# flanglet/kanzi-go

Measured on AMD Instinct MI355X. Metric: encode+decode MB/s (round trip of the whole stream, uncompressed 10^6 B per second), higher is better.
Workload: dtype u8

## Files before the change

### kanzi-go_amd/csrc/ans1.hip

```cpp
#include "bits.h"

#define KNZ_ANS1_CHUNK (4u << 20)
#define KNZ_ANS1_LR 11
#define KNZ_ANS1_SCALE 2048
#define KNZ_ANS1_LDS_MAX_CHUNKS 1280u
#define KNZ_ANS1_CTXHDR_BYTES 448
#define KNZ_ANS1_U0_CAP (256 * KNZ_ANS1_CTXHDR_BYTES + 64)
#define KNZ_ANS1_U1_OFF KNZ_ANS1_U0_CAP
#define KNZ_ANS1_PAY_OFF (KNZ_ANS1_U0_CAP + 64)
#define KNZ_ANS1_PAY_CAP (((KNZ_ANS1_CHUNK / 8) * 11) + 64)
#define KNZ_ANS1_SLOT (KNZ_ANS1_PAY_OFF + KNZ_ANS1_PAY_CAP + 64)
#define KNZ_ANS1_CUM_STRIDE 257
#define KNZ_ANS1_PAYRING 8192
#define KNZ_ANS1_RING 2048

struct Ans1Args {
    const uint64_t* blk_off;
    const uint32_t* blk_len;
    uint32_t chunks_per_block;
    uint32_t nslots;
    uint8_t* scratch;
    uint32_t* unit_bits;
    uint32_t* unit_src;
    uint32_t* freqs;
// ... 397 lines not shown
        flushed += c0 + c1 + c2;
        wave_sync_lds();
    };
#pragma unroll
    for (int j = 0; j < KNZ_ANS1_GROUP; j++) { buf0[j].x = 0; buf0[j].y = 0xFFFFFFFFu; buf0[j].z = 0; buf0[j].w = 0; buf1[j] = buf0[j]; }
    for (uint32_t t0 = 0; t0 < steps + 2 * KNZ_ANS1_GROUP && steps; t0 += 3 * KNZ_ANS1_GROUP) {
        load_group(t0, buf2, xm2); knz_a1e_run_group<0>(st, buf0, mine);
        const uint32_t f0 = xm0;
        load_group(t0 + KNZ_ANS1_GROUP, buf0, xm0); knz_a1e_run_group<1>(st, buf1, mine);
        const uint32_t f1 = xm1;
        load_group(t0 + 2 * KNZ_ANS1_GROUP, buf1, xm1); knz_a1e_run_group<2>(st, buf2, mine);
        flush(f0, f1, xm2);
    }
    const uint32_t s1 = wave_shfl(st, 1), s2 = wave_shfl(st, 2), s3 = wave_shfl(st, 3);
    if (bad && lane == 0) a.blk_status[b] = KNZ_ERR_PROCESS_BLOCK;
    if (live && lane == 0) {
        const uint32_t end4 = n & ~3u;
        const uint32_t tail = n & 3;
        for (uint32_t i = 0; i < tail; i++) payEnd[i] = src[end4 + i];
        const uint32_t nbytes = 2 * flushed + tail;
        uint32_t w[8];
        for (int i = 0; i < 8; i++) w[i] = 0;
        KnzBitWriter bw;
        bw.init(w);
        knz_put_varint(bw, nbytes);
        bw.put(st, 32); bw.put(s1, 32); bw.put(s2, 32); bw.put(s3, 32);
        uint32_t* u1 = (uint32_t*)(slot + KNZ_ANS1_U1_OFF);
        for (int i = 0; i < 8; i++) u1[i] = knz_bswap32(w[i]);
        uint32_t* ubits = a.unit_bits + (size_t)slotId * KNZ_UNITS_PER_CHUNK;
        uint32_t* usrc = a.unit_src + (size_t)slotId * KNZ_UNITS_PER_CHUNK;
        ubits[1] = bw.pos;
        ubits[2] = 8 * nbytes;
        usrc[2] = (uint32_t)(KNZ_ANS1_PAY_OFF + KNZ_ANS1_PAY_CAP - 2 * flushed);
    }
}
#endif

struct Ans1DecArgs {
    const uint8_t* stream; uint64_t nbytes;
    const uint32_t* blk_pre_len;
    const uint8_t* blk_mode;
    const uint64_t* chunk_bit;
    const uint64_t* blk_out_off;
    uint32_t chunks_per_block;
    uint32_t nslots;
    uint32_t* dtab;
    uint32_t* info;
    uint64_t* paybit;
    int32_t* blk_status;
    uint32_t plain_loop;
    uint64_t* progress;
};

template <typename R>
__device__ static bool knz_ans1_parse_ctx(R& r, uint16_t* f, uint32_t llr, uint32_t scale, int& countOut) {
    uint8_t alpha[256];
    int count = 0;
    if (r.read(1) == 0) {
        if (r.read(1) == 1) count = 0;
        else { count = 256; if (f) for (int i = 0; i < 256; i++) alpha[i] = (uint8_t)i; }
    } else {
        const uint32_t lastMask = r.read(5);
        if (f) {
            for (uint32_t mm = 0; mm <= lastMask; mm++) {
                const uint32_t mask = r.read(8);
                for (int j = 0; j < 8; j++) if ((mask >> j) & 1) alpha[count++] = (uint8_t)(8 * mm + j);
            }
        } else {
            for (uint32_t bitsLeft = 8 * (lastMask + 1); bitsLeft > 0;) {
                const uint32_t take = bitsLeft > 32 ? 32 : bitsLeft;
                count += __popc(r.read(take));
                bitsLeft -= take;
            }
        }
    }
    countOut = count;
    if (count == 0) return true;
    const int chk = count < 64 ? 6 : 8;
    uint32_t sum = 0;
    for (int i = 1; i < count; i += chk) {
        const uint32_t logMax = r.read(llr);
        if ((1u << logMax) > scale) return false;
        const int endj = min(i + chk, count);
        if (!f) { r.skip_bits((uint32_t)(endj - i) * logMax); continue; }
        for (int j = i; j < endj; j++) {
            uint32_t fr = 1;
            if (logMax > 0) { fr = 1 + r.read(logMax); if (fr >= scale) return false; }
            f[alpha[j]] = (uint16_t)fr;
            sum += fr;
        }
    }
    if (f) {
        if (scale <= sum) return false;
        f[alpha[0]] = (uint16_t)(scale - sum);
    }
    return true;
}

template <typename R>
__device__ static bool knz_ans1_parse_header(R& r, uint16_t* freq16, uint32_t& lrOut, int& totalAlpha, uint64_t* ctxpos, bool store) {
    const uint32_t lr = 8 + r.read(3);
    lrOut = lr;
    if (lr > 16) return false;
    uint32_t llr = 3;
    while ((1u << llr) <= lr) llr++;
    const uint32_t scale = 1u << lr;
    totalAlpha = 0;
    for (int k = 0; k < 256; k++) {
        if (ctxpos && store) ctxpos[k] = r.tell();
        int count = 0;
        if (!knz_ans1_parse_ctx(r, freq16 ? freq16 + (size_t)k * 256 : nullptr, llr, scale, count)) return false;
        totalAlpha += count;
    }
    if (ctxpos && store) ctxpos[256] = r.tell();
    return true;
}

__global__ __launch_bounds__(256) void knz_ans1_dec_tables_kernel(Ans1DecArgs a, uint16_t* freq16, uint16_t* cum16, const uint64_t* ctx_bit) {
    __shared__ int s_mode;
    __shared__ uint32_t s_lr;
    __shared__ int s_total, s_badctx;
    const int tid = threadIdx.x;
    const uint32_t slotId = blockIdx.x;
    const uint32_t b = slotId / a.chunks_per_block, k = slotId % a.chunks_per_block;
    uint32_t* info = a.info + (size_t)slotId * 8;
    const uint32_t preLen = a.blk_pre_len[b];
    if (tid == 0) info[0] = 0;
    if (a.blk_status[b] != 0 || (uint64_t)k * KNZ_ANS1_CHUNK >= preLen) return;
    if ((a.blk_mode[b] & 0x80) || preLen <= 32) { if (tid == 0) info[0] = 1; return; }
    uint16_t* f16 = freq16 + (size_t)slotId * 65536;
    for (int i = tid; i < 65536; i += 256) f16[i] = 0;
    __syncthreads();
    const uint64_t* cpos = ctx_bit ? ctx_bit + (size_t)slotId * 257 : nullptr;
    if (cpos) {
        if (tid == 0) { s_total = 0; s_badctx = 0; }
        __syncthreads();
        KnzStreamReader r0;
// ... 550 lines not shown
```

### kanzi-go_amd/csrc/huffman_dec.hip

```cpp
#include "bits.h"

struct KnzStreamReader {
    const uint32_t* words;
    uint64_t nwords;
    uint64_t next;
    uint64_t win;
    uint32_t navail;
    uint32_t pre;
    __device__ __forceinline__ uint32_t ld_raw(uint64_t i) const { return i < nwords ? words[i] : 0u; }
    __device__ __forceinline__ uint32_t ld(uint64_t i) const { return knz_bswap32(ld_raw(i)); }
    __device__ __forceinline__ void init(const uint8_t* base, uint64_t nbytes, uint64_t bitpos) {
        words = (const uint32_t*)base;
        nwords = (nbytes + 3) >> 2;
        uint64_t q = bitpos >> 5;
        uint32_t off = (uint32_t)(bitpos & 31);
        win = ((uint64_t)ld(q) << 32) | ld(q + 1);
        win <<= off;
        navail = 64 - off;
        next = q + 2;
        pre = ld_raw(next);
    }
    __device__ __forceinline__ void refill() {
        if (navail <= 32) { win |= (uint64_t)knz_bswap32(pre) << (32 - navail); navail += 32; next++; pre = ld_raw(next); }
    }
    __device__ __forceinline__ uint32_t peek(uint32_t n) { refill(); return (uint32_t)(win >> (64 - n)); }
    __device__ __forceinline__ void skip(uint32_t n) { refill(); win <<= n; navail -= n; }
    __device__ __forceinline__ void consume(uint32_t n) { win <<= n; navail -= n; }
    __device__ __forceinline__ void skip_bits(uint32_t n) { if (n <= 32) skip(n); else seek(tell() + n); }
    __device__ __forceinline__ uint32_t read(uint32_t n) { uint32_t v = peek(n); win <<= n; navail -= n; return v; }
    __device__ __forceinline__ uint64_t tell() const { return (next << 5) - navail; }
    __device__ __forceinline__ void seek(uint64_t bitpos) { init((const uint8_t*)words, nwords << 2, bitpos); }
};

struct KnzWaveReader {
    const uint32_t* words;
    uint64_t nwords;
    uint64_t base;
    uint32_t w0, w1;
    uint64_t next;
    uint64_t win;
    uint32_t navail;
    __device__ __forceinline__ void stage(uint64_t b) {
        const uint64_t l = (uint64_t)lane_id();
        base = b;
        w0 = (b + l < nwords) ? words[b + l] : 0u;
        w1 = (b + 64 + l < nwords) ? words[b + 64 + l] : 0u;
    }
    __device__ __forceinline__ uint32_t ld(uint64_t i) {
        if (i < base || i >= base + 128) stage(i);
        const uint32_t k = (uint32_t)(i - base);
        const uint32_t v = k < 64 ? wave_readlane(w0, k) : wave_readlane(w1, k - 64);
        return knz_bswap32(v);
    }
    __device__ __forceinline__ void init(const uint8_t* b, uint64_t nbytes, uint64_t bitpos) {
        words = (const uint32_t*)b;
        nwords = (nbytes + 3) >> 2;
        stage(bitpos >> 5);
        seek(bitpos);
    }
    __device__ __forceinline__ void seek(uint64_t bitpos) {
        const uint64_t q = bitpos >> 5;
        const uint32_t off = (uint32_t)(bitpos & 31);
        win = ((uint64_t)ld(q) << 32) | ld(q + 1);
        win <<= off;
        navail = 64 - off;
        next = q + 2;
    }
    __device__ __forceinline__ void refill() {
        if (navail <= 32) { win |= (uint64_t)ld(next++) << (32 - navail); navail += 32; }
    }
    __device__ __forceinline__ uint32_t peek(uint32_t n) { refill(); return (uint32_t)(win >> (64 - n)); }
    __device__ __forceinline__ void skip(uint32_t n) { refill(); win <<= n; navail -= n; }
    __device__ __forceinline__ void skip_bits(uint32_t n) { if (n <= 32) skip(n); else seek(tell() + n); }
    __device__ __forceinline__ uint32_t read(uint32_t n) { uint32_t v = peek(n); win <<= n; navail -= n; return v; }
    __device__ __forceinline__ uint64_t tell() const { return (next << 5) - navail; }
};

template <typename R>
__device__ __forceinline__ uint32_t knz_read_varint(R& r) {
    uint32_t res = 0, shift = 0;
    for (int i = 0; i < 4; i++) {
        uint32_t v = r.read(8);
        res |= (v & 0x7F) << shift;
        if (v < 128) return res;
        shift += 7;
    }
    uint32_t v = r.read(8);
    return res | ((v & 0x0F) << 28);
}

template <typename R>
__device__ static bool knz_ans1_parse_header(R& r, uint16_t* freq16, uint32_t& lrOut, int& totalAlpha, uint64_t* ctxpos, bool store);

struct WalkStreamArgs {
    const uint8_t* stream; uint64_t nbytes;
    uint64_t first_bit;
    uint64_t seg_bits;
    uint32_t max_blocks;
    uint64_t* blk_bit;
    uint64_t* blk_bits;
    uint32_t* result;
};

__global__ void knz_dec_walk_stream_kernel(WalkStreamArgs a) {
    if (threadIdx.x != 0 || blockIdx.x != 0) return;
    KnzStreamReader r;
    r.init(a.stream, a.nbytes, a.first_bit);
    const uint64_t limit = a.nbytes << 3;
    uint32_t n = 0, err = 0;
    for (;;) {
        if (a.seg_bits && r.tell() >= a.first_bit + a.seg_bits) break;
        if (r.tell() + 8 > limit) { err = KNZ_ERR_PROCESS_BLOCK; break; }
        uint32_t lr = r.read(5) + 3;
        uint64_t read = 0;
        if (lr > 32) { read = (uint64_t)r.read(lr - 32) << 32; read |= r.read(32); }
        else read = r.read(lr);
        if (read == 0) break;
        if (read > ((uint64_t)1 << 34)) { err = KNZ_ERR_BLOCK_SIZE; break; }
        uint64_t pos = r.tell();
        if (pos + read > limit) { err = KNZ_ERR_PROCESS_BLOCK; break; }
        if (n >= a.max_blocks) { err = KNZ_ERR_BLOCK_SIZE; break; }
        a.blk_bit[n] = pos;
        a.blk_bits[n] = read;
        n++;
        r.seek(pos + read);
    }
    a.result[0] = n;
    a.result[1] = err;
// ... 16 lines not shown
    if (threadIdx.x != 0 || blockIdx.x != 0) return;
    KnzStreamReader r;
    r.init(a.stream, a.nbytes, a.first_bit);
    const uint64_t limit = a.nbytes << 3;
    uint64_t id = a.first_id, n = 0, end = 0;
    uint32_t seen = 0, err = 0;
    while (id < a.to) {
        const uint64_t at = r.tell();
        if (at + 8 > limit) { err = KNZ_ERR_PROCESS_BLOCK; break; }
        const uint32_t lr = r.read(5) + 3;
        uint64_t read = 0;
        if (lr > 32) { read = (uint64_t)r.read(lr - 32) << 32; read |= r.read(32); }
        else read = r.read(lr);
        const uint64_t pos = r.tell();
        if (read == 0) { end = pos; if (a.hinted && seen == 0) err = KNZ_ERR_PROCESS_BLOCK; break; }
        if (read > ((uint64_t)1 << 34)) { err = KNZ_ERR_BLOCK_SIZE; break; }
        if (pos + read > limit) { err = KNZ_ERR_PROCESS_BLOCK; break; }
        if (seen >= a.max_blocks) { err = KNZ_ERR_BLOCK_SIZE; break; }
        seen++;
        if (id >= a.from) {
            if (n < a.cap) { a.blk_bit[n * a.stride] = a.frames ? at : pos; a.blk_bits[n * a.stride] = read; }
            n++;
        }
        id++;
        r.seek(pos + read);
    }
    a.result[0] = n;
    a.result[1] = err;
    a.result[2] = end;
}

struct WalkBlocksArgs {
    const uint8_t* stream; uint64_t nbytes;
    const uint64_t* blk_bit; const uint64_t* blk_bits;
    uint32_t nblocks;
    uint32_t block_size;
    uint32_t checksum_bits;
    uint32_t entropy;
    uint32_t chunks_per_block;
    uint32_t payload_only;
    uint32_t given_len;
    uint32_t* blk_pre_len;
    uint8_t* blk_mode;
    uint8_t* blk_skip;
    uint64_t* blk_cksum;
    uint64_t* chunk_bit;
    int32_t* blk_status;
    uint64_t* blk_end_bit;
    uint32_t check_out;
    uint64_t* out_off;
    uint64_t out_base, out_stride, out_cap;
    uint32_t stream_block_size;
    uint64_t* ans1_ctx_bit;
};

template <typename R>
__device__ __forceinline__ void knz_skip_expg(R& r) {
    uint32_t w = r.peek(17);
    if (w & 0x10000) { r.skip(1); return; }
    if (w == 0) { r.skip(17); return; }
    uint32_t z = (uint32_t)__builtin_clz(w << 15);
    uint32_t lg = z & 7;
    r.skip(z + 1);
    r.skip(lg + 1);
}

#define KNZ_EXPG_WIN 12
__device__ __forceinline__ uint32_t knz_expg_lut_entry(uint32_t w) {
    uint32_t pos = 0, codes = 0;
    while (pos < KNZ_EXPG_WIN) {
        if ((w >> (KNZ_EXPG_WIN - 1 - pos)) & 1) { codes++; pos++; continue; }
        uint32_t z = 0;
        while (pos + z < KNZ_EXPG_WIN && !((w >> (KNZ_EXPG_WIN - 1 - pos - z)) & 1)) z++;
        if (pos + z >= KNZ_EXPG_WIN) break;
        const uint32_t total = z + 1 + (z & 7) + 1;
        if (pos + total > KNZ_EXPG_WIN) break;
        codes++; pos += total;
    }
    return (codes << 4) | pos;
}

struct HufDecArgs {
    const uint8_t* stream; uint64_t nbytes;
    const uint32_t* blk_pre_len;
    const uint8_t* blk_mode;
    const uint64_t* chunk_bit;
    const uint64_t* blk_out_off;
    uint32_t chunks_per_block;
    uint32_t entropy;
    uint8_t* out;
    int32_t* blk_status;
};

__global__ __launch_bounds__(64) void knz_huf_decode_kernel(HufDecArgs a, const uint8_t* only) {
    __shared__ uint16_t s_table[1 << KNZ_HUF_MAXLEN];
    __shared__ uint8_t s_len[256];
    __shared__ uint8_t s_alpha[256];
    __shared__ uint16_t s_C[256];
    __shared__ uint8_t s_symAt[256];
    __shared__ uint32_t s_fragbits[4];
    __shared__ uint64_t s_fragpos[4];
    __shared__ int s_count, s_err;
    __shared__ uint64_t s_tailpos;

    const int lane = threadIdx.x;
    if (only && !only[blockIdx.x]) return;
// ... 153 lines not shown
```

### kanzi-go_amd/csrc/huffman_par.hip

```cpp
#include "bits.h"

#ifdef KNZ_PROFILE_PHASES
__device__ unsigned long long g_knz_prof[32];
#define KNZ_PROF_T(var) const unsigned long long var = __builtin_readcyclecounter()
#define KNZ_PROF_ADD(i, a, b) do { if (threadIdx.x == 0) atomicAdd(&g_knz_prof[i], (b) - (a)); } while (0)
#define KNZ_PROF_INC(i, v) do { if (threadIdx.x == 0) atomicAdd(&g_knz_prof[i], (unsigned long long)(v)); } while (0)
#else
#define KNZ_PROF_INC(i, v)
#define KNZ_PROF_T(var)
#define KNZ_PROF_ADD(i, a, b)
#endif

#define KNZ_HUF_SYNC_BITS 192
#define KNZ_HUF_LANE_CAP 84
#define KNZ_HW_WORDS 136

struct KnzHufHdr {
    uint32_t count;
    uint32_t fb[4];
    uint32_t end;
    uint32_t status;
};

struct KnzLinWin {
// ... 564 lines not shown
        const uint32_t nchunks = (preLen + chunkSize - 1) / chunkSize;
        if (nchunks > cpb) status = KNZ_ERR_BLOCK_SIZE;
        const uint32_t* swords = (const uint32_t*)a.stream;
        const uint64_t snwords = (a.nbytes + 3) >> 2;
        uint64_t pos = r.tell();
        bool stale = false;
        uint32_t filled = 0;
        for (uint32_t k = 0; k < nchunks && status == 0; k++) {
            const uint32_t sz = min(chunkSize, preLen - k * chunkSize);
            if (writer) knz_publish64(&a.chunk_bit[(size_t)b * cpb + k], pos);
            published = k + 1;
            if (entropy == KNZ_E_HUFFMAN && sz >= 32 && ringLive) {
                KNZ_PROF_T(w0);
                const uint64_t w0i = pos >> 5;
                const uint32_t rel = (uint32_t)(w0i - ringOrigin);
                if (writer) vsync[1] = rel;
                const uint32_t need = (uint32_t)min((uint64_t)rel + KNZ_HW_WORDS, ((snwords - ringOrigin + 255) & ~(uint64_t)255));
                if (filled < need) {
                    uint32_t spins = 0;
                    while ((filled = vsync[0]) < need) { wave_spin_pause(); if (++spins > (1u << 24)) break; }
                    if (filled < need) ringLive = false;
                    else wg_fence_acquire();
                }
              if (ringLive) {
                KNZ_PROF_T(w1);
                KNZ_PROF_T(w2);
                const KnzHufHdr hdr = knz_huf_parse_header_wave<false>(KnzRingWin{s_ring, rel, KNZ_WALK_RING - 1}, (uint32_t)(pos & 31), nullptr, nullptr, (int)threadIdx.x);
                KNZ_PROF_T(w3);
                KNZ_PROF_T(w4);
                KNZ_PROF_ADD(8, w0, w1); KNZ_PROF_ADD(9, w1, w2); KNZ_PROF_ADD(10, w2, w3); KNZ_PROF_ADD(11, w3, w4);
                if (hdr.status == 2) { status = KNZ_ERR_PROCESS_BLOCK; break; }
                if (hdr.status == 0) {
                    uint64_t np = (w0i << 5) + hdr.end;
                    if (hdr.count > 1) {
                        if ((int32_t)(hdr.fb[0] | hdr.fb[1] | hdr.fb[2] | hdr.fb[3]) < 0) status = KNZ_ERR_PROCESS_BLOCK;
                        np += (uint64_t)hdr.fb[0] + hdr.fb[1] + hdr.fb[2] + hdr.fb[3] + 8ull * (sz & 3);
                    }
                    pos = np;
                    stale = true;
                    if (pos > limit) status = KNZ_ERR_PROCESS_BLOCK;
                    continue;
                }
              }
            }
            if (stale) { r.seek(pos); stale = false; }
            if (entropy == KNZ_E_NONE || (entropy == KNZ_E_HUFFMAN && sz < 32) || ((entropy == KNZ_E_ANS0 || entropy == KNZ_E_ANS1) && preLen <= 32)) {
                r.seek(r.tell() + 8ull * sz);
            } else if (entropy == KNZ_E_FPAQ) {
                const uint32_t szb = knz_read_varint(r);
                if ((int32_t)szb < 0 || (uint64_t)szb >= 2ull * preLen) status = KNZ_ERR_PROCESS_BLOCK;
                r.seek(r.tell() + 56 + 8ull * szb);
            } else if (entropy == KNZ_E_ANS1) {
                uint32_t lr; int total;
                if (!knz_ans1_parse_header(r, nullptr, lr, total, a.ans1_ctx_bit ? a.ans1_ctx_bit + ((size_t)b * cpb + k) * 257 : nullptr, writer) || total == 0) { status = KNZ_ERR_PROCESS_BLOCK; break; }
                const uint32_t szb = knz_read_varint(r);
                if (szb >= (1u << 27)) status = KNZ_ERR_PROCESS_BLOCK;
                r.seek(r.tell() + 128 + 8ull * szb);
            } else if (entropy == KNZ_E_ANS0) {
                const uint32_t lr = 8 + r.read(3);
                uint32_t llr = 3;
                while ((1u << llr) <= lr) llr++;
                uint32_t count;
                if (r.read(1) == 0) count = r.read(1) == 1 ? 0 : 256;
                else {
                    uint32_t lastMask = r.read(5);
                    count = 0;
                    for (uint32_t m = 0; m <= lastMask; m++) count += (uint32_t)__popc(r.read(8));
                }
                if (count == 0) { status = KNZ_ERR_PROCESS_BLOCK; break; }
                const uint32_t chk = count < 64 ? 6 : 8;
                for (uint32_t i = 1; i < count; i += chk) {
                    const uint32_t logMax = r.read(llr);
                    const uint32_t endj = min(i + chk, count);
                    if (logMax > 16) { status = KNZ_ERR_PROCESS_BLOCK; break; }
                    r.seek(r.tell() + (uint64_t)(endj - i) * logMax);
                }
                if (count > 1 && status == 0) {
                    const uint32_t szb = knz_read_varint(r);
                    if (szb >= (1u << 27)) status = KNZ_ERR_PROCESS_BLOCK;
                    r.seek(r.tell() + 128 + 8ull * szb);
                }
            } else {
                uint32_t count;
                if (r.read(1) == 0) {
                    if (r.read(1) == 1) { status = KNZ_ERR_PROCESS_BLOCK; break; }
                    count = 256;
                } else {
                    uint32_t lastMask = r.read(5);
                    count = 0;
                    for (uint32_t bitsLeft = 8 * (lastMask + 1); bitsLeft > 0;) {
                        const uint32_t take = bitsLeft > 32 ? 32 : bitsLeft;
                        count += (uint32_t)__popc(r.read(take));
                        bitsLeft -= take;
                    }
                    if (count == 0) { status = KNZ_ERR_PROCESS_BLOCK; break; }
                }
                for (uint32_t i = 0; i < count;) {
                    const uint32_t e = s_lut[r.peek(KNZ_EXPG_WIN)];
                    const uint32_t nc = e >> 4;
                    if (nc == 0 || i + nc > count) { knz_skip_expg(r); i++; }
                    else { r.skip(e & 15); i += nc; }
                }
                if (count > 1) {
                    uint64_t fb = 0;
                    for (int j = 0; j < 4; j++) {
                        uint32_t v = knz_read_varint(r);
                        if ((int32_t)v < 0) status = KNZ_ERR_PROCESS_BLOCK;
                        fb += v;
                    }
                    r.seek(r.tell() + fb + 8ull * (sz & 3));
// ... 56 lines not shown
```

### kanzi-go_amd/csrc/knz_batch.inc

```

struct EncodeBatch {
    const uint8_t* d_src; uint64_t n;
    uint8_t* d_dst; uint64_t dst_cap;
    int framed = 0, with_header = 0, with_end = 0; int64_t header_input_size = 0;
    uint64_t out_stride = 0;
    int payload_only = 0;
    int keep_probes = 0;
    uint64_t total_bits = 0;
    struct Many { const ManyStream* streams = nullptr; uint32_t n_streams = 0, blocks = 0, max_len = 0; uint32_t* blk_stream = nullptr; } many;
    static EncodeBatch stream(const uint8_t* src, uint64_t n, uint8_t* dst, uint64_t cap, int64_t header_input_size) {
        EncodeBatch eb = segment(src, n, dst, cap); eb.with_header = eb.with_end = 1; eb.header_input_size = header_input_size; return eb;
    }
    static EncodeBatch segment(const uint8_t* src, uint64_t n, uint8_t* dst, uint64_t cap) { EncodeBatch eb(src, n, dst, cap); eb.framed = 1; return eb; }
    static EncodeBatch block_streams(const uint8_t* src, uint64_t n, uint8_t* dst, uint64_t stride, uint64_t count) {
        EncodeBatch eb(src, n, dst, stride * count + 64); eb.out_stride = stride; return eb;
    }
    static EncodeBatch payload(const uint8_t* src, uint64_t n, uint8_t* dst, uint64_t cap) { EncodeBatch eb = block_streams(src, n, dst, cap, 1); eb.payload_only = 1; return eb; }
private:
    EncodeBatch(const uint8_t* src, uint64_t nn, uint8_t* dst, uint64_t cap) : d_src(src), n(nn), d_dst(dst), dst_cap(cap) {}
};

struct DecodeBatch {
    const uint8_t* d_stream; uint64_t nbytes;
    int framed;
// ... 529 lines not shown
        WalkRangeArgs wr;
        wr.stream = db.d_stream; wr.nbytes = db.nbytes; wr.first_bit = db.first_bit; wr.first_id = db.rg_first_id; wr.from = db.rg_from; wr.to = db.rg_to;
        wr.max_blocks = walkBound; wr.cap = maxBlocks; wr.frames = 0; wr.stride = 1; wr.hinted = db.rg_hinted ? 1 : 0;
        wr.blk_bit = blkBit.as<uint64_t>(); wr.blk_bits = blkBits.as<uint64_t>(); wr.result = h->total_bits.as<uint64_t>();
        hipLaunchKernelGGL(knz_dec_walk_range_kernel, dim3(1), dim3(1), 0, st, wr);
        uint64_t* res = (uint64_t*)h->pinned;
        HIP_OK(hipMemcpyAsync(res, h->total_bits.p, 24, hipMemcpyDeviceToHost, st));
        HIP_OK(hipStreamSynchronize(st));
        if (res[1]) return knz_set_error(h, (int)res[1], "invalid block framing in stream");
        nblocks = (uint32_t)res[0];
    } else if (db.framed) {
        WalkStreamArgs ws;
        ws.stream = db.d_stream; ws.nbytes = db.nbytes; ws.first_bit = db.first_bit; ws.seg_bits = db.seg_bits; ws.max_blocks = maxBlocks;
        ws.blk_bit = blkBit.as<uint64_t>(); ws.blk_bits = blkBits.as<uint64_t>(); ws.result = h->total_bits.as<uint32_t>();
        hipLaunchKernelGGL(knz_dec_walk_stream_kernel, dim3(1), dim3(1), 0, st, ws);
        uint32_t* res = (uint32_t*)h->pinned;
        HIP_OK(hipMemcpyAsync(res, h->total_bits.p, 8, hipMemcpyDeviceToHost, st));
        HIP_OK(hipStreamSynchronize(st));
        if (res[1]) return knz_set_error(h, (int)res[1], "invalid block framing in stream");
        nblocks = res[0];
    }
    db.nblocks = nblocks;
    db.total_out = 0;
    db.pre_len.assign(nblocks, 0); db.end_bit.assign(nblocks, 0); db.status.assign(nblocks, 0);
    return KNZ_OK;
}

static int dec_header_pass(Handle* h, DecStage& d, const EntropyCodec& ec, hipStream_t st) {
    const DecodeBatch& db = d.db;
    const uint32_t nblocks = d.nblocks = db.nblocks;
    WalkBlocksArgs& wb = d.wb;
    const uint32_t maxPre = db.payload_only ? db.given_len : knz_max_encoded_len(db.transform, db.block_size);
    const uint32_t cpb = d.cpb = std::max<uint32_t>(1, (maxPre + ec.chunk - 1) / ec.chunk);
    const size_t nslots = d.nslots = (size_t)nblocks * cpb;
    if (h->blk_len.reserve(4 * (size_t)nblocks) || h->blk_skip.reserve(2 * (size_t)nblocks + 16) || h->blk_cksum.reserve(8 * (size_t)nblocks) ||
        h->chunk_rel.reserve(8 * nslots) || h->blk_status.reserve(4 * (size_t)nblocks) || h->blk_off.reserve(8 * (size_t)nblocks) ||
        h->dec_tables.reserve(8 * (size_t)nblocks))
        return knz_set_error(h, KNZ_ERR_CREATE_DECOMPRESSOR, "device workspace allocation failed");
    hipEventRecord(h->ev[0], st);
    wb.stream = db.d_stream; wb.nbytes = db.nbytes; wb.blk_bit = h->blk_dst_bit.as<uint64_t>(); wb.blk_bits = h->blk_written.as<uint64_t>();
    wb.nblocks = nblocks;
    wb.block_size = db.block_size + std::max<uint32_t>(512, db.block_size >> 4);
    wb.checksum_bits = db.checksum_bits; wb.entropy = db.entropy; wb.chunks_per_block = cpb;
    wb.payload_only = db.payload_only; wb.given_len = db.given_len;
    wb.blk_pre_len = h->blk_len.as<uint32_t>(); wb.blk_mode = h->blk_skip.as<uint8_t>(); wb.blk_skip = h->blk_skip.as<uint8_t>() + nblocks;
    wb.blk_cksum = h->blk_cksum.as<uint64_t>(); wb.chunk_bit = h->chunk_rel.as<uint64_t>(); wb.blk_status = h->blk_status.as<int32_t>();
    wb.blk_end_bit = h->dec_tables.as<uint64_t>();
    const bool fusedWalk = d.fusedWalk = (db.entropy == KNZ_E_HUFFMAN || db.entropy == KNZ_E_ANS0) && knz_test_switch("KNZ_HUF_SPLIT_WALK") == nullptr;
    d.xf = db.transform != 0 && !db.payload_only;
    const bool direct = d.direct = fusedWalk && !d.xf;
    wb.check_out = direct ? 1 : 0; wb.out_off = h->blk_off.as<uint64_t>(); wb.out_base = (uint64_t)db.d_out; wb.out_stride = db.out_stride;
    wb.out_cap = db.out_cap; wb.stream_block_size = db.block_size;
    wb.ans1_ctx_bit = nullptr;
    if (db.entropy == KNZ_E_ANS1) {
        if (h->a1_ctxpos.reserve((size_t)nslots * 257 * 8 + 64)) return knz_set_error(h, KNZ_ERR_CREATE_DECOMPRESSOR, "device workspace allocation failed");
        wb.ans1_ctx_bit = h->a1_ctxpos.as<uint64_t>();
    }
    if (fusedWalk) hipLaunchKernelGGL(knz_dec_block_headers_kernel, dim3(nblocks), dim3(64), 0, st, wb);
    else hipLaunchKernelGGL(knz_dec_walk_blocks_kernel, dim3(nblocks), dim3(128), 0, st, wb);
    hipEventRecord(h->ev[1], st);
    return KNZ_OK;
}

static int dec_block_fits(Handle* h, const DecodeBatch& db, uint32_t b) {
    if (db.pre_len[b] > db.block_size || (db.pre_len[b] > db.out_stride && b + 1 < db.nblocks))
        return knz_set_error(h, KNZ_ERR_PROCESS_BLOCK, "block decodes to more than the stream block size");
    if ((uint64_t)b * db.out_stride + db.pre_len[b] > db.out_cap) return knz_set_error(h, KNZ_ERR_WRITE_FILE, "destination buffer too small");
    return KNZ_OK;
}

static int dec_place_outputs(Handle* h, DecStage& d, hipStream_t st) {
    DecodeBatch& db = d.db;
    XfBatch& xb = d.xb;
    const uint32_t nblocks = d.nblocks;
    const bool xf = d.xf;
    uint64_t& xstride = d.xstride;
    if (xf) {
        const uint64_t padded = (uint64_t)db.block_size + std::max<uint32_t>(512, db.block_size >> 4);
        xstride = (std::max<uint64_t>(knz_max_encoded_len(db.transform, db.block_size), padded) + 64 + 15) & ~(uint64_t)15;
        if (xf_alloc(h, xb, nblocks, xstride)) return knz_set_error(h, KNZ_ERR_CREATE_DECOMPRESSOR, "device workspace allocation failed");
        xb.ctx_entropy = db.entropy; xb.ctx_block_size = db.block_size;
    }
    std::vector<uint64_t> off(nblocks);
    for (uint32_t b = 0; b < nblocks; b++) off[b] = xf ? (uint64_t)h->xf_r1.p + (uint64_t)b * xstride : (uint64_t)db.d_out + (uint64_t)b * db.out_stride;
    HIP_OK(hipMemcpyAsync(h->blk_off.p, off.data(), 8 * (size_t)nblocks, hipMemcpyHostToDevice, st));
    HIP_OK(hipMemcpyAsync(db.pre_len.data(), h->blk_len.p, 4 * (size_t)nblocks, hipMemcpyDeviceToHost, st));
    HIP_OK(hipMemcpyAsync(db.status.data(), h->blk_status.p, 4 * (size_t)nblocks, hipMemcpyDeviceToHost, st));
    HIP_OK(hipStreamSynchronize(st));
    int first = KNZ_OK;
    for (uint32_t b = 0; b < nblocks; b++) {
        int rc = KNZ_OK;
        if (db.status[b]) rc = knz_set_error(h, db.status[b], "invalid block in stream");
        else if (xf) { if (db.pre_len[b] > xstride) rc = knz_set_error(h, KNZ_ERR_BLOCK_SIZE, "block larger than the decoder buffers"); }
        else rc = dec_block_fits(h, db, b);
        if (rc && db.block_failed(b, rc, first)) return rc;
    }
    return first;
}

static int dec_inverse_transforms(Handle* h, DecStage& d, hipStream_t st) {
    DecodeBatch& db = d.db;
    XfBatch& xb = d.xb;
    const RankPipe& pipe = d.pipe;
    const uint32_t nblocks = d.nblocks;
    if (!pipe.on) {
        std::vector<uint8_t> ones(nblocks, 1);
// ... 89 lines not shown
```

### kanzi-go_amd/csrc/wave.h

```cpp
#pragma once
#include <hip/hip_runtime.h>
#include <stdint.h>

#define KNZ_WAVE 64

#ifndef KNZ_HIP_EMU
#if defined(__HIP_DEVICE_COMPILE__) && !defined(__gfx950__)
#error "libknz_gpu is written for gfx950 (MI355X) only: --offload-arch=gfx950"
#endif
__device__ __forceinline__ int lane_id() { return (int)__builtin_amdgcn_mbcnt_hi(~0u, __builtin_amdgcn_mbcnt_lo(~0u, 0u)); }
__device__ __forceinline__ uint32_t wave_shfl(uint32_t v, int src) { return (uint32_t)__shfl((int)v, src, 64); }
__device__ __forceinline__ uint64_t wave_shfl64(uint64_t v, int src) {
    uint32_t lo = wave_shfl((uint32_t)v, src), hi = wave_shfl((uint32_t)(v >> 32), src);
    return ((uint64_t)hi << 32) | lo;
}
__device__ __forceinline__ uint64_t wave_ballot(bool p) { return __ballot(p); }
__device__ __forceinline__ uint32_t wave_bcast(uint32_t v, int src) { return (uint32_t)__builtin_amdgcn_readlane((int)v, src); }
__device__ __forceinline__ uint32_t wave_readlane(uint32_t v, uint32_t src) {
    return (uint32_t)__builtin_amdgcn_readlane((int)v, (int)__builtin_amdgcn_readfirstlane((int)src));
}
__device__ __forceinline__ void wave_sync() {
    __builtin_amdgcn_fence(__ATOMIC_RELEASE, "workgroup");
    __builtin_amdgcn_wave_barrier();
    __builtin_amdgcn_fence(__ATOMIC_ACQUIRE, "workgroup");
}
__device__ __forceinline__ uint32_t wave_shr1(uint32_t v) { return (uint32_t)__builtin_amdgcn_mov_dpp((int)v, 0x138, 0xF, 0xF, true); }
__device__ __forceinline__ uint32_t wave_ror1(uint32_t v) { return (uint32_t)__builtin_amdgcn_mov_dpp((int)v, 0x13C, 0xF, 0xF, true); }
__device__ __forceinline__ uint32_t wave_shl1(uint32_t v) { return (uint32_t)__builtin_amdgcn_mov_dpp((int)v, 0x130, 0xF, 0xF, true); }
__device__ __forceinline__ uint32_t wave_writelane0(uint32_t v, uint32_t val) {
    const int sv = __builtin_amdgcn_readfirstlane((int)val);
    asm("v_writelane_b32 %0, %1, 0" : "+v"(v) : "s"(sv));
    return v;
}
template <int L> __device__ __forceinline__ uint32_t wave_writelane_at(uint32_t v, uint32_t val) {
    const int sv = __builtin_amdgcn_readfirstlane((int)val);
    asm("v_writelane_b32 %0, %1, %2" : "+v"(v) : "s"(sv), "n"(L));
    return v;
}
__device__ __forceinline__ uint32_t wave_shr1_old(uint32_t v, uint32_t old) { return (uint32_t)__builtin_amdgcn_update_dpp((int)old, (int)v, 0x138, 0xF, 0xF, false); }
__device__ __forceinline__ uint32_t wave_shr1_keep0(uint32_t cur, uint32_t v) { return (uint32_t)__builtin_amdgcn_update_dpp((int)cur, (int)v, 0x138, 0xF, 0xF, false); }
__device__ __forceinline__ uint32_t wave_in_vgpr(uint32_t x) { asm("" : "+v"(x)); return x; }
__device__ __forceinline__ void wave_rank_fused(int q, uint32_t e, uint32_t vnew, int vqc, uint32_t& t, int& m) {
    t = vnew; m = vqc;
    int mx;
    asm volatile("v_max_i32_dpp %2, %3, %5 wave_shr:1 row_mask:0xf bank_mask:0xf\n\t"
                 "v_cmp_gt_i32_e32 vcc, %2, %5\n\t"
                 "v_cndmask_b32_dpp %0, %4, %0, vcc wave_shr:1 row_mask:0xf bank_mask:0xf\n\t"
                 "v_min_i32_dpp %1, %3, %1 wave_shr:1 row_mask:0xf bank_mask:0xf"
                 : "+v"(t), "+v"(m), "=&v"(mx) : "v"(q), "v"(e), "v"(vqc) : "vcc");
}
template <int L>
__device__ __forceinline__ void wave_rank_step_packed(uint32_t& e, int& q, uint32_t& ob, uint32_t r, uint32_t vi8, uint32_t vff, uint32_t lane, uint32_t vmax) {
    uint32_t se, vnew;
    int qx, vqc;
    uint64_t keep;
    asm volatile("v_readlane_b32 %[se], %[e], %[r]\n\t"
                 "v_cmp_ge_u32_e32 vcc, %[r], %[lane]\n\t"
                 "v_cndmask_b32_e32 %[qx], %[vmax], %[q], vcc\n\t"
                 "v_add_u32_e32 %[vqc], %[se], %[vi8]\n\t"
                 "v_lshrrev_b32_e32 %[vqc], 9, %[vqc]\n\t"
                 "v_and_or_b32 %[vnew], %[se], %[vff], %[vi8]\n\t"
                 "v_cmp_gt_i32_e64 %[keep], %[qx], %[vqc]\n\t"
                 "v_max_i32_dpp %[qx], %[q], %[vqc] wave_shr:1 row_mask:0xf bank_mask:0xf\n\t"
                 "v_cmp_gt_i32_e32 vcc, %[qx], %[vqc]\n\t"
                 "v_cndmask_b32_dpp %[vnew], %[e], %[vnew], vcc wave_shr:1 row_mask:0xf bank_mask:0xf\n\t"
                 "v_min_i32_dpp %[vqc], %[q], %[vqc] wave_shr:1 row_mask:0xf bank_mask:0xf\n\t"
                 "v_cndmask_b32_e64 %[e], %[vnew], %[e], %[keep]\n\t"
                 "v_cndmask_b32_e64 %[q], %[vqc], %[q], %[keep]\n\t"
                 "v_writelane_b32 %[ob], %[se], %[L]"
                 : [e] "+v"(e), [q] "+v"(q), [ob] "+v"(ob), [se] "=&s"(se), [vnew] "=&v"(vnew), [qx] "=&v"(qx), [vqc] "=&v"(vqc), [keep] "=&s"(keep)
                 : [r] "s"(r), [vi8] "v"(vi8), [vff] "v"(vff), [lane] "v"(lane), [vmax] "v"(vmax), [L] "n"(L)
                 : "vcc");
}
__device__ __forceinline__ uint32_t knz_lds_addr(const void* p) { return (uint32_t)(uintptr_t)(__attribute__((address_space(3))) const char*)p; }
__device__ __forceinline__ uint64_t wave_sload_u64_async(const uint8_t* p) { uint64_t v; asm volatile("s_load_dwordx2 %0, %1, 0x0" : "=&s"(v) : "s"(p) : "memory"); return v; }
__device__ __forceinline__ uint32_t wave_sload_u32_async(const uint8_t* p) { uint32_t v; asm volatile("s_load_dword %0, %1, 0x0" : "=&s"(v) : "s"(p) : "memory"); return v; }
#define WAVE_SLOAD_WAIT7(a, b, c, d, e, f, g) asm volatile("s_waitcnt lgkmcnt(0)" : "+s"(a), "+s"(b), "+s"(c), "+s"(d), "+s"(e), "+s"(f), "+s"(g))
#define WAVE_SLOAD_WAIT5A(a, b, c, d, e, p0, p1, p2, p3, p4) \
    asm volatile("s_waitcnt lgkmcnt(0)" : "+s"(a), "+s"(b), "+s"(c), "+s"(d), "+s"(e) : "s"(p0), "s"(p1), "s"(p2), "s"(p3), "s"(p4))
__device__ __forceinline__ uint32_t wave_pin_sgpr(uint32_t x) { asm volatile("" : "+s"(x)); return x; }
template <int L> __device__ __forceinline__ uint32_t wave_writelane_c(uint32_t v, uint32_t val) {
    const int sv = __builtin_amdgcn_readfirstlane((int)val);
    asm("v_writelane_b32 %0, %1, %2" : "+v"(v) : "s"(sv), "n"(L));
    return v;
}
typedef uint32_t knz_u32x4 __attribute__((ext_vector_type(4)));
typedef knz_u32x4 knz_u32x4_a4 __attribute__((aligned(4)));
__device__ __forceinline__ uint32_t wave_sload_u32(const uint8_t* p) { return *(const __attribute__((address_space(4))) uint32_t*)(uintptr_t)p; }
struct WaveLzLoads { knz_u32x4 a; uint32_t c, d; uint64_t e, f; };
__device__ __forceinline__ WaveLzLoads wave_lz_step_loads(const uint8_t* src, const uint8_t* cand, const uint8_t* cp, uint32_t o0, uint32_t o2, uint32_t o3, uint32_t o4, uint32_t o5) {
    WaveLzLoads r;
    asm volatile("s_load_dwordx4 %0, %5, %8\n\t"
                 "s_load_dword %1, %6, %9\n\t"
                 "s_load_dword %2, %7, %10\n\t"
// ... 40 lines not shown
inline void knz_scalar_cache_inv() {}
inline void wg_fence_acquire() {}
inline void knz_publish64(uint64_t* p, uint64_t v) { *(volatile uint64_t*)p = v; }
inline uint64_t knz_poll64(const uint64_t* p) { return *(const volatile uint64_t*)p; }
inline void wg_spin_pause() { hipemu::spin_pause(); }
inline uint64_t knz_realtime() { static uint64_t t = 0; return t += 1000; }
inline void wave_order_lanes() { hipemu::wave_barrier(); }
inline int32_t knz_wg_load_i32(const int32_t* p) { return *(const volatile int32_t*)p; }
inline int32_t knz_agent_load_i32(const int32_t* p) { return *(const volatile int32_t*)p; }
inline void knz_wg_max_i32(int32_t* p, int32_t v) { if (*(volatile int32_t*)p < v) *(volatile int32_t*)p = v; }
inline void wave_raise_priority() {}
inline uint32_t knz_byte_perm(uint32_t hi, uint32_t lo, uint32_t sel) {
    const uint64_t both = ((uint64_t)hi << 32) | lo;
    uint32_t r = 0;
    for (int i = 0; i < 4; i++) r |= (uint32_t)((both >> (8 * ((sel >> (8 * i)) & 7u))) & 0xFFu) << (8 * i);
    return r;
}
inline uint32_t knz_mul24(uint32_t a, uint32_t b) { return (a & 0xFFFFFFu) * (b & 0xFFFFFFu); }
inline uint32_t wave_uniform(uint32_t v) { return v; }
inline int lane_id() { return hipemu::lane(); }
inline uint64_t wave_shfl64(uint64_t v, int src) {
    uint64_t* s = hipemu::wave_slots();
    s[hipemu::lane()] = v;
    hipemu::wave_barrier();
    uint64_t r = s[src & 63];
    hipemu::wave_barrier();
    return r;
}
inline uint32_t wave_shfl(uint32_t v, int src) { return (uint32_t)wave_shfl64(v, src); }
inline uint64_t wave_ballot(bool p) {
    uint64_t* s = hipemu::wave_slots();
    s[hipemu::lane()] = p ? 1 : 0;
    hipemu::wave_barrier();
    uint64_t r = 0;
    for (int i = 0; i < 64; i++) r |= (s[i] & 1) << i;
    hipemu::wave_barrier();
    return r;
}
inline uint32_t wave_bcast(uint32_t v, int src) { return wave_shfl(v, src); }
inline uint32_t wave_mbcnt64(uint64_t m) { return (uint32_t)__builtin_popcountll(m & ((1ull << hipemu::lane()) - 1)); }
inline uint32_t wave_quad_xor1(uint32_t v) { return wave_shfl(v, hipemu::lane() ^ 1); }
inline uint32_t wave_quad_xor2(uint32_t v) { return wave_shfl(v, hipemu::lane() ^ 2); }
inline uint32_t wave_readlane(uint32_t v, uint32_t src) { return wave_shfl(v, (int)src); }
inline void wave_sync() { hipemu::wave_barrier(); }
inline void wave_sync_lds() { hipemu::wave_barrier(); }
inline uint32_t wave_shr1(uint32_t v) { const uint32_t r = wave_shfl(v, hipemu::lane() - 1); return hipemu::lane() == 0 ? 0u : r; }
inline uint32_t wave_ror1(uint32_t v) { return wave_shfl(v, (hipemu::lane() + 63) & 63); }
inline uint32_t wave_writelane0(uint32_t v, uint32_t val) { return hipemu::lane() == 0 ? val : v; }
template <int L> inline uint32_t wave_writelane_at(uint32_t v, uint32_t val) { return hipemu::lane() == L ? val : v; }
inline uint32_t wave_shl1(uint32_t v) { const uint32_t r = wave_shfl(v, hipemu::lane() + 1); return hipemu::lane() == 63 ? 0u : r; }
inline uint32_t wave_shr1_old(uint32_t v, uint32_t old) { const uint32_t r = wave_shfl(v, hipemu::lane() - 1); return hipemu::lane() == 0 ? old : r; }
inline uint32_t wave_shr1_keep0(uint32_t cur, uint32_t v) { const uint32_t r = wave_shfl(v, hipemu::lane() - 1); return hipemu::lane() == 0 ? cur : r; }
inline uint32_t wave_in_vgpr(uint32_t x) { return x; }
inline void wave_rank_fused(int q, uint32_t e, uint32_t vnew, int vqc, uint32_t& t, int& m) {
    const int qp = (int)wave_shfl((uint32_t)q, hipemu::lane() - 1);
    const uint32_t ep = wave_shfl(e, hipemu::lane() - 1);
    if (hipemu::lane() == 0) { t = vnew; m = vqc; } else { t = qp > vqc ? vnew : ep; m = qp < vqc ? qp : vqc; }
}
template <int L>
inline void wave_rank_step_packed(uint32_t& e, int& q, uint32_t& ob, uint32_t r, uint32_t vi8, uint32_t vff, uint32_t lane, uint32_t vmax) {
    const uint32_t se = wave_shfl(e, (int)r);
    const int vqc = (int)((se + vi8) >> 9);
    const uint32_t vnew = (se & vff) | vi8;
    const int qx = lane > r ? (int)vmax : q;
    const bool keep = qx > vqc;
    uint32_t t; int m;
    wave_rank_fused(q, e, vnew, vqc, t, m);
    e = keep ? e : t;
    q = keep ? q : m;
    if ((int)lane == L) ob = se;
}
inline uint32_t wave_pin_sgpr(uint32_t x) { return x; }
inline uint64_t wave_sload_u64_async(const uint8_t* p) { uint64_t v; __builtin_memcpy(&v, p, 8); return v; }
inline uint32_t wave_sload_u32_async(const uint8_t* p) { uint32_t v; __builtin_memcpy(&v, p, 4); return v; }
#define WAVE_SLOAD_WAIT7(a, b, c, d, e, f, g) do { } while (0)
#define WAVE_SLOAD_WAIT5A(a, b, c, d, e, p0, p1, p2, p3, p4) do { } while (0)
template <int L> inline uint32_t wave_writelane_c(uint32_t v, uint32_t val) { return hipemu::lane() == L ? val : v; }
struct knz_u32x4 { uint32_t x, y, z, w; };
inline uint32_t wave_sload_u32(const uint8_t* p) { uint32_t v; __builtin_memcpy(&v, p, 4); return v; }
inline knz_u32x4 wave_sload_u32x4(const uint8_t* p) { knz_u32x4 v; __builtin_memcpy(&v, p, 16); return v; }
struct WaveLzLoads { knz_u32x4 a; uint32_t c, d; uint64_t e, f; };
inline WaveLzLoads wave_lz_step_loads(const uint8_t* src, const uint8_t* cand, const uint8_t* cp, uint32_t o0, uint32_t o2, uint32_t o3, uint32_t o4, uint32_t o5) {
    WaveLzLoads r;
    __builtin_memcpy(&r.a, src + o0, 16); __builtin_memcpy(&r.c, cand + o2, 4); __builtin_memcpy(&r.d, cp + o3, 4);
    __builtin_memcpy(&r.e, src + o4, 8); __builtin_memcpy(&r.f, src + o5, 8);
    return r;
}
#endif

#ifndef KNZ_HIP_EMU
__device__ __forceinline__ uint32_t wave_scan_incl(uint32_t v) {
    v += (uint32_t)__builtin_amdgcn_update_dpp(0, (int)v, 0x111, 0xF, 0xF, false);
    v += (uint32_t)__builtin_amdgcn_update_dpp(0, (int)v, 0x112, 0xF, 0xF, false);
    v += (uint32_t)__builtin_amdgcn_update_dpp(0, (int)v, 0x114, 0xF, 0xF, false);
    v += (uint32_t)__builtin_amdgcn_update_dpp(0, (int)v, 0x118, 0xF, 0xF, false);
    v += (uint32_t)__builtin_amdgcn_update_dpp(0, (int)v, 0x142, 0xA, 0xF, false);
    v += (uint32_t)__builtin_amdgcn_update_dpp(0, (int)v, 0x143, 0xC, 0xF, false);
    return v;
}
#else
__device__ __forceinline__ uint32_t wave_scan_incl(uint32_t v) {
    int l = lane_id();
#pragma unroll
    for (int d = 1; d < 64; d <<= 1) {
        uint32_t t = wave_shfl(v, l - d);
        if (l >= d) v += t;
// ... 15 lines not shown
```

Before: 387.2.

## Walk ANS1 headers with a wave-cooperative prefetching bit reader

Adds KnzPosReader, a bit reader in which each lane of the wave holds one stream word in registers. Peeks become readlane operations plus a position counter, and each refill prefetches the next 63 words in parallel, so the header walk no longer issues a dependent global load at every refill. The ANS1 context skip path is also restructured: it checks the maximum logMax once at the end instead of per group, and the group loop is specialised at compile time for groups of 6 or 8. The serial reader stays reachable through an environment switch, at the cost of more register pressure and extra wave-wide loads on refill.

```diff
diff --git a/kanzi-go_amd/csrc/ans1.hip b/kanzi-go_amd/csrc/ans1.hip
--- a/kanzi-go_amd/csrc/ans1.hip
+++ b/kanzi-go_amd/csrc/ans1.hip
@@ -473,6 +473,17 @@
     uint64_t* progress;
 };
 
+template <uint32_t CHK, typename R>
+__device__ __forceinline__ uint32_t knz_ans1_skip_groups(R& r, uint32_t llr, uint32_t& left) {
+    uint32_t widest = 0;
+    for (; left >= CHK; left -= CHK) {
+        const uint32_t logMax = r.read(llr);
+        widest = max(widest, logMax);
+        r.skip_bits(CHK * logMax);
+    }
+    return widest;
+}
+
 template <typename R>
 __device__ static bool knz_ans1_parse_ctx(R& r, uint16_t* f, uint32_t llr, uint32_t scale, int& countOut) {
     uint8_t alpha[256];
@@ -498,12 +509,21 @@
     countOut = count;
     if (count == 0) return true;
     const int chk = count < 64 ? 6 : 8;
+    if (!f) {
+        uint32_t left = (uint32_t)count - 1u;
+        uint32_t widest = chk == 8 ? knz_ans1_skip_groups<8>(r, llr, left) : knz_ans1_skip_groups<6>(r, llr, left);
+        if (left != 0) {
+            const uint32_t logMax = r.read(llr);
+            widest = max(widest, logMax);
+            r.skip_bits(left * logMax);
+        }
+        return (1u << widest) <= scale;
+    }
     uint32_t sum = 0;
     for (int i = 1; i < count; i += chk) {
         const uint32_t logMax = r.read(llr);
         if ((1u << logMax) > scale) return false;
         const int endj = min(i + chk, count);
-        if (!f) { r.skip_bits((uint32_t)(endj - i) * logMax); continue; }
         for (int j = i; j < endj; j++) {
             uint32_t fr = 1;
             if (logMax > 0) { fr = 1 + r.read(logMax); if (fr >= scale) return false; }
diff --git a/kanzi-go_amd/csrc/huffman_dec.hip b/kanzi-go_amd/csrc/huffman_dec.hip
--- a/kanzi-go_amd/csrc/huffman_dec.hip
+++ b/kanzi-go_amd/csrc/huffman_dec.hip
@@ -74,6 +74,53 @@
     __device__ __forceinline__ void skip_bits(uint32_t n) { if (n <= 32) skip(n); else seek(tell() + n); }
     __device__ __forceinline__ uint32_t read(uint32_t n) { uint32_t v = peek(n); win <<= n; navail -= n; return v; }
     __device__ __forceinline__ uint64_t tell() const { return (next << 5) - navail; }
+};
+
+struct KnzPosReader {
+    const uint32_t* words;
+    uint64_t nwords;
+    uint64_t base;
+    uint32_t p;
+    uint32_t hi, lo;
+    uint32_t nhi, nlo;
+    __device__ __forceinline__ void load_raw(uint64_t b, uint32_t ln, uint32_t& h, uint32_t& l) const {
+        const uint64_t i = b + ln;
+        h = i < nwords ? words[i] : 0u;
+        l = i + 1 < nwords ? words[i + 1] : 0u;
+    }
+    __device__ __forceinline__ void init(const uint8_t* b, uint64_t nbytes, uint64_t bitpos) {
+        words = (const uint32_t*)b;
+        nwords = (nbytes + 3) >> 2;
+        base = bitpos >> 5;
+        p = wave_uniform((uint32_t)(bitpos & 31)) + 63 * 32;
+        load_raw(base, (uint32_t)lane_id(), nhi, nlo);
+        base -= 63;
+        advance();
+    }
+    __device__ __forceinline__ void advance() {
+        if ((p >> 5) >= 126) {
+            const uint64_t t = tell();
+            base = (t >> 5) - 63;
+            p = (uint32_t)(t & 31) + 63 * 32;
+            load_raw(base + 63, (uint32_t)lane_id(), nhi, nlo);
+        }
+        hi = knz_bswap32(nhi); lo = knz_bswap32(nlo);
+        base += 63; p -= 63 * 32;
+        uint32_t ln = (uint32_t)lane_id();
+        wave_tie3(hi, lo, ln);
+        load_raw(base + 63, ln, nhi, nlo);
+    }
+    __device__ __forceinline__ uint32_t peek(uint32_t n) {
+        if (__builtin_expect((p >> 5) >= 63, 0)) advance();
+        const uint32_t k = p >> 5;
+        const uint64_t w = ((uint64_t)wave_readlane(hi, k) << 32) | wave_readlane(lo, k);
+        return (uint32_t)((w << (p & 31)) >> (64 - n));
+    }
+    __device__ __forceinline__ void skip(uint32_t n) { p += n; }
+    __device__ __forceinline__ void consume(uint32_t n) { p += n; }
+    __device__ __forceinline__ void skip_bits(uint32_t n) { p += n; }
+    __device__ __forceinline__ uint32_t read(uint32_t n) { const uint32_t v = wave_pin_sgpr(peek(n)); p += n; return v; }
+    __device__ __forceinline__ uint64_t tell() const { return (base << 5) + p; }
 };
 
 template <typename R>
@@ -196,6 +243,7 @@
     uint64_t out_base, out_stride, out_cap;
     uint32_t stream_block_size;
     uint64_t* ans1_ctx_bit;
+    uint32_t ans1_serial_walk;
 };
 
 template <typename R>
diff --git a/kanzi-go_amd/csrc/huffman_par.hip b/kanzi-go_amd/csrc/huffman_par.hip
--- a/kanzi-go_amd/csrc/huffman_par.hip
+++ b/kanzi-go_amd/csrc/huffman_par.hip
@@ -640,10 +640,20 @@
                 r.seek(r.tell() + 56 + 8ull * szb);
             } else if (entropy == KNZ_E_ANS1) {
                 uint32_t lr; int total;
-                if (!knz_ans1_parse_header(r, nullptr, lr, total, a.ans1_ctx_bit ? a.ans1_ctx_bit + ((size_t)b * cpb + k) * 257 : nullptr, writer) || total == 0) { status = KNZ_ERR_PROCESS_BLOCK; break; }
-                const uint32_t szb = knz_read_varint(r);
-                if (szb >= (1u << 27)) status = KNZ_ERR_PROCESS_BLOCK;
-                r.seek(r.tell() + 128 + 8ull * szb);
+                uint64_t* ctxpos = a.ans1_ctx_bit ? a.ans1_ctx_bit + ((size_t)b * cpb + k) * 257 : nullptr;
+                if (!a.ans1_serial_walk) {
+                    KnzPosReader pr;
+                    pr.init(a.stream, a.nbytes, r.tell());
+                    if (!knz_ans1_parse_header(pr, nullptr, lr, total, ctxpos, writer) || total == 0) { status = KNZ_ERR_PROCESS_BLOCK; break; }
+                    const uint32_t szb = knz_read_varint(pr);
+                    if (szb >= (1u << 27)) status = KNZ_ERR_PROCESS_BLOCK;
+                    r.seek(pr.tell() + 128 + 8ull * szb);
+                } else {
+                    if (!knz_ans1_parse_header(r, nullptr, lr, total, ctxpos, writer) || total == 0) { status = KNZ_ERR_PROCESS_BLOCK; break; }
+                    const uint32_t szb = knz_read_varint(r);
+                    if (szb >= (1u << 27)) status = KNZ_ERR_PROCESS_BLOCK;
+                    r.seek(r.tell() + 128 + 8ull * szb);
+                }
             } else if (entropy == KNZ_E_ANS0) {
                 const uint32_t lr = 8 + r.read(3);
                 uint32_t llr = 3;
diff --git a/kanzi-go_amd/csrc/knz_batch.inc b/kanzi-go_amd/csrc/knz_batch.inc
--- a/kanzi-go_amd/csrc/knz_batch.inc
+++ b/kanzi-go_amd/csrc/knz_batch.inc
@@ -605,6 +605,7 @@
     wb.check_out = direct ? 1 : 0; wb.out_off = h->blk_off.as<uint64_t>(); wb.out_base = (uint64_t)db.d_out; wb.out_stride = db.out_stride;
     wb.out_cap = db.out_cap; wb.stream_block_size = db.block_size;
     wb.ans1_ctx_bit = nullptr;
+    wb.ans1_serial_walk = knz_test_switch("KNZ_ANS1_SERIAL_WALK") != nullptr ? 1u : 0u;
     if (db.entropy == KNZ_E_ANS1) {
         if (h->a1_ctxpos.reserve((size_t)nslots * 257 * 8 + 64)) return knz_set_error(h, KNZ_ERR_CREATE_DECOMPRESSOR, "device workspace allocation failed");
         wb.ans1_ctx_bit = h->a1_ctxpos.as<uint64_t>();
diff --git a/kanzi-go_amd/csrc/wave.h b/kanzi-go_amd/csrc/wave.h
--- a/kanzi-go_amd/csrc/wave.h
+++ b/kanzi-go_amd/csrc/wave.h
@@ -40,6 +40,7 @@
 __device__ __forceinline__ uint32_t wave_shr1_old(uint32_t v, uint32_t old) { return (uint32_t)__builtin_amdgcn_update_dpp((int)old, (int)v, 0x138, 0xF, 0xF, false); }
 __device__ __forceinline__ uint32_t wave_shr1_keep0(uint32_t cur, uint32_t v) { return (uint32_t)__builtin_amdgcn_update_dpp((int)cur, (int)v, 0x138, 0xF, 0xF, false); }
 __device__ __forceinline__ uint32_t wave_in_vgpr(uint32_t x) { asm("" : "+v"(x)); return x; }
+__device__ __forceinline__ void wave_tie3(uint32_t& a, uint32_t& b, uint32_t& c) { asm volatile("" : "+v"(a), "+v"(b), "+v"(c)); }
 __device__ __forceinline__ void wave_rank_fused(int q, uint32_t e, uint32_t vnew, int vqc, uint32_t& t, int& m) {
     t = vnew; m = vqc;
     int mx;
@@ -186,6 +187,7 @@
 inline uint32_t wave_shr1_old(uint32_t v, uint32_t old) { const uint32_t r = wave_shfl(v, hipemu::lane() - 1); return hipemu::lane() == 0 ? old : r; }
 inline uint32_t wave_shr1_keep0(uint32_t cur, uint32_t v) { const uint32_t r = wave_shfl(v, hipemu::lane() - 1); return hipemu::lane() == 0 ? cur : r; }
 inline uint32_t wave_in_vgpr(uint32_t x) { return x; }
+inline void wave_tie3(uint32_t&, uint32_t&, uint32_t&) {}
 inline void wave_rank_fused(int q, uint32_t e, uint32_t vnew, int vqc, uint32_t& t, int& m) {
     const int qp = (int)wave_shfl((uint32_t)q, hipemu::lane() - 1);
     const uint32_t ep = wave_shfl(e, hipemu::lane() - 1);
```

After: 389.2 (median of 6 runs). No clear change (+0.5%).
